# Leo-Liao-Chao/Uncertainty-Aware-CILQR-for-Trajectory-Optimization

Hardware: AMD Instinct MI355X
Metric: CILQR solves/sec (N=50, batch B) (higher is better)
Workload: dtype f64

## Files before the change

### uncertainty-aware-cilqr-for-trajectory-optimization_amd/csrc/cilqr_api.cpp

```cpp
#include <math.h>
#include <stdarg.h>
#include <stdio.h>
#include <stdlib.h>
#include <string.h>

#include <new>
#include <string>
#include <vector>

#include "cilqr_internal.h"

#include "cilqr_handle.h"

namespace cilqr {
thread_local std::string g_last_error;

int fail(int code, const char* fmt, ...) {
  char buf[512];
  va_list ap;
  va_start(ap, fmt);
  vsnprintf(buf, sizeof(buf), fmt, ap);
  va_end(ap);
  g_last_error = buf;
  return code;
// ... 2 lines not shown

using cilqr::fail;

namespace {

void derive(const cilqr_params& p, cilqr::KParams& k) {
  k.dt = p.timestep;
  k.desired_speed = p.desired_speed;
  k.tolerance = p.tolerance;
  k.w_acc = p.w_acc; k.w_yawrate = p.w_yawrate; k.w_pos = p.w_pos; k.w_vel = p.w_vel; k.w_obstacle = p.w_obstacle;
  k.q1_acc = p.q1_acc; k.q2_acc = p.q2_acc; k.q1_yawrate = p.q1_yawrate; k.q2_yawrate = p.q2_yawrate;
  k.q1_front = p.q1_front; k.q2_front = p.q2_front; k.q1_rear = p.q1_rear; k.q2_rear = p.q2_rear;
  k.acc_max = p.acc_max; k.acc_min = p.acc_min;
  k.yaw_hi = tan(p.steer_angle_max) / p.wheelbase;
  k.yaw_lo = tan(p.steer_angle_min) / p.wheelbase;
  k.half_dt2 = p.timestep * p.timestep / 2.0;
  k.wheelbase = p.wheelbase; k.speed_max = p.speed_max;
  k.t_safe = p.t_safe; k.s_safe_a = p.s_safe_a; k.s_safe_b = p.s_safe_b;
  k.ego_rad = p.ego_rad; k.ego_front = p.ego_front; k.ego_rear = p.ego_rear;
  k.lamb_factor = p.lamb_factor; k.lamb_max = p.lamb_max;
  k.max_iterations = p.max_iterations;
  k.n_samples = p.num_of_local_wpts * 10;
}

int check_sizes(const cilqr_handle* h, int B, int N, int M) {
  if (!h) return fail(CILQR_ERR_ARG, "null handle");
  if (B < 0 || B > h->max_batch) return fail(CILQR_ERR_ARG, "B=%d outside [0,%d]", B, h->max_batch);
  if (N < 1 || N > h->max_horizon) return fail(CILQR_ERR_ARG, "N=%d outside [1,%d]", N, h->max_horizon);
  if (M < 0 || M > h->max_obstacles) return fail(CILQR_ERR_ARG, "M=%d outside [0,%d]", M, h->max_obstacles);
  return CILQR_OK;
}

cilqr::SolveKnobs read_knobs(int simds) {
  const auto on = [](const char* name) { return getenv(name) != nullptr ? 1 : 0; };
  const auto num = [](const char* name, int unset) { const char* v = getenv(name); return v ? atoi(v) : unset; };
  cilqr::SolveKnobs k = {};
  k.simds = simds; k.force_g = num("CILQR_FORCE_G", 0);
  k.hint_off = on("CILQR_NO_SCHEDULE_HINT"); k.pair_on = on("CILQR_PAIR_KERNEL"); k.steal_off = on("CILQR_NO_LANE_SHARING"); k.split_off = on("CILQR_NO_SPLIT_KERNEL");
  k.share_off = on("CILQR_NO_SHARE_KERNEL"); k.tab_budget_kb = num("CILQR_LDS_TABLE_KB", 0);
  k.split_w = num("CILQR_SPLIT_W", 0);
  if (on("CILQR_SHARE_W")) k.share_w = num("CILQR_SHARE_W", 0) == 3 ? 3 : 2;
  k.share_max = num("CILQR_SHARE_MAX_B", -1);
  return k;
}

cilqr::SolveArgs handle_args(const cilqr_handle* h, int B, int N, int M, uint32_t flags) {
  cilqr::SolveArgs a = {};
  a.obs_tab = h->d_obs_tab; a.fwd = h->d_ws;
  a.redo = h->d_redo; a.diag = h->diag; a.passes = h->passes; a.unc = h->unc; a.kp = h->kp;
  a.B = B; a.N = N; a.M = M; a.flags = flags;
  return a;
}

template <typename T>
hipError_t dmalloc(T** p, size_t n) {
  *p = nullptr;
  if (n == 0) return hipSuccess;
  return hipMalloc((void**)p, n * sizeof(T));
}

int grow(float** p, size_t* cap, size_t n) {
  if (n <= *cap) return CILQR_OK;
  if (*p) HIP_TRY(hipFree(*p));
  *p = nullptr; *cap = 0;
  HIP_TRY(dmalloc(p, n));
  *cap = n;
  return CILQR_OK;
}

void set_obstacles(cilqr::SolveArgs& s, int M, const cilqr_obstacles* obs) {
  if (M <= 0) return;
  s.obs_pose = obs->pose; s.obs_dim = obs->dim; s.obs_weight = obs->weight;
  s.obs_bs = obs->batch_stride; s.obs_ms = obs->obstacle_stride; s.obs_ts = obs->step_stride; s.obs_wbs = obs->weight_batch_stride;
}

int check_sampled(const cilqr_handle* h, const char* name, int B, int N, int n_obs, int n_samples) {
  if (n_obs < 1 || n_samples < 2) return fail(CILQR_ERR_ARG, "%s: needs n_obs >= 1 and n_samples >= 2", name);
  if ((long)n_obs * n_samples > 1 << 20) return fail(CILQR_ERR_ARG, "%s: n_obs * n_samples too large", name);
  return check_sizes(h, B, N, n_obs * n_samples);
}

}

static int launch_wave_scheduled(cilqr_handle* h, cilqr::SolveArgs& a, const cilqr::WavePlan& plan, void* stream) {
  a.order = plan.hinted && h->hint_B == a.B && h->hint_stream == stream ? h->d_order : nullptr;
  a.hint_passes = plan.hinted ? h->d_hint_passes : nullptr;
  HIP_TRY(cilqr::launch_solve_wave(a, plan, (hipStream_t)stream));
  if (plan.hinted) {
    HIP_TRY(cilqr::launch_schedule_order(h->d_hint_passes, a.B, h->d_order, (hipStream_t)stream));
    h->hint_B = a.B; h->hint_stream = stream;
  }
  return CILQR_OK;
}

namespace {

int check_obstacles(int B, int N, int M, const cilqr_obstacles* o, size_t* span, size_t* w_span) {
  if (span) *span = 0;
  if (w_span) *w_span = 0;
  if (M == 0) return CILQR_OK;
  if (!o) return fail(CILQR_ERR_ARG, "cilqr_solve_batch_obstacles: M = %d but obs is null", M);
  if (!o->pose || !o->dim) return fail(CILQR_ERR_ARG, "cilqr_solve_batch_obstacles: M > 0 but obs->pose or obs->dim is null");
  if (o->batch_stride < 0 || o->obstacle_stride < 0 || o->step_stride < 0 || o->weight_batch_stride < 0)
    return fail(CILQR_ERR_ARG, "cilqr_solve_batch_obstacles: negative stride");
  const int64_t lim = (int64_t)1 << 40;
  if (o->batch_stride > lim || o->obstacle_stride > lim || o->step_stride > lim || o->weight_batch_stride > lim)
    return fail(CILQR_ERR_ARG, "cilqr_solve_batch_obstacles: stride beyond 2^40 entries");
  const int64_t b1 = B > 0 ? B - 1 : 0;
  if (span) *span = (size_t)(b1 * o->batch_stride + (int64_t)(M - 1) * o->obstacle_stride + (int64_t)(N - 1) * o->step_stride + 1);
  if (w_span && o->weight) *w_span = (size_t)(b1 * o->weight_batch_stride + M);
  return CILQR_OK;
}

int solve_device(cilqr_handle* h, void* stream, int B, int N, int M, const double* x0, double* U, const double* poly,
                 const double* xplan_fl, const cilqr_obstacles& o, double* X_out, double* J_out, int32_t* iters_out,
                 int32_t* status_out, uint32_t flags) {
  cilqr::SolveArgs a = handle_args(h, B, N, M, flags);
  a.x0 = x0; a.U = U; a.poly = poly; a.xplan_fl = xplan_fl;
  set_obstacles(a, M, &o);
  a.obs_shared = M > 0 && B > 1 && o.batch_stride == 0 && (!a.obs_weight || o.weight_batch_stride == 0) ? 1 : 0;
  a.X_out = X_out; a.J_out = J_out; a.iters_out = iters_out; a.status_out = status_out;
  a.steal = h->knobs.steal_off ? 0 : 1;
  HIP_TRY(hipSetDevice(h->device));
  const int G = cilqr::plan_group_lanes(h->knobs, B, N, M);
  if (G != 64) { HIP_TRY(cilqr::launch_solve_groups(a, G, h->d_ws, (hipStream_t)stream)); return CILQR_OK; }
  const cilqr::WavePlan plan = cilqr::plan_wave(h->knobs, {B, N, M, 0, h->kp.n_samples, flags, h->unc.layer != nullptr, a.obs_shared != 0});
  if (plan.too_large)
    return fail(CILQR_ERR_UNSUPPORTED, "cilqr_solve_batch: horizon %d needs %zu bytes of LDS per solve (limit %zu)", N, plan.lds_general, cilqr::SOLVE_LDS_MAX);
  return launch_wave_scheduled(h, a, plan, stream);
}

}

extern "C" {

int cilqr_abi_version(void) { return CILQR_ABI_VERSION; }

int cilqr_device_count(void) {
  int count = 0;
  if (hipGetDeviceCount(&count) != hipSuccess) return 0;
  int usable = 0;
  for (int d = 0; d < count; ++d) {
    hipDeviceProp_t prop;
    if (hipGetDeviceProperties(&prop, d) == hipSuccess && strncmp(prop.gcnArchName, "gfx950", 6) == 0) ++usable;
  }
  return usable;
}

const char* cilqr_last_error(void) { return cilqr::g_last_error.c_str(); }

void cilqr_params_default(cilqr_params* p) {
  if (!p) return;
  memset(p, 0, sizeof(*p));
  p->num_of_local_wpts = 20; p->poly_order = 5; p->desired_speed = 5.0;
  p->timestep = 0.1; p->horizon = 40; p->tolerance = 1e-4; p->max_iterations = 20;
  p->num_states = 4; p->num_ctrls = 2;
  p->w_acc = 1.0; p->w_yawrate = 4.0; p->w_pos = 0.65; p->w_vel = 3.0; p->w_obstacle = 1.0; p->w_uncertainty = 1.0;
  p->q1_acc = 1.0; p->q2_acc = 1.0; p->q1_yawrate = 1.0; p->q2_yawrate = 1.0;
  p->q1_front = 2.75; p->q2_front = 2.75; p->q1_rear = 2.5; p->q2_rear = 2.5;
  p->q1_uncertainty = 2.5; p->q2_uncertainty = 2.5;
  p->acc_max = 2.0; p->acc_min = -5.5; p->steer_angle_min = -0.75; p->steer_angle_max = 0.75;
  p->wheelbase = 2.94; p->speed_max = 30.0;
  p->steer_control_max = 1.0; p->steer_control_min = -1.0;
  p->throttle_control_max = 1.0; p->throttle_control_min = -1.0;
  p->t_safe = 0.1; p->s_safe_a = 0; p->s_safe_b = 0; p->ego_rad = 1.35;
  p->ego_front = 1.47 + 0.925; p->ego_rear = 1.47 + 0.925;
  p->length = 4.79; p->width = 2.16; p->safe_length = 0.0; p->safe_width = 0.0;
  p->lamb_factor = 10; p->lamb_max = 10000;
}

int cilqr_default_control_seq(int N, double* U) {
  if (N < 1 || !U) return fail(CILQR_ERR_ARG, "cilqr_default_control_seq: bad argument");
  const int num_zeros = N / 2;
  for (int i = 0; i < N; ++i) {
    U[2 * i] = 0.5;
    U[2 * i + 1] = i < num_zeros ? 0.0 : 0.1;
  }
  return CILQR_OK;
}

int cilqr_create(const cilqr_params* p, int max_batch, int max_horizon, int max_obstacles, int device,
                 cilqr_handle** out) {
  if (!p || !out) return fail(CILQR_ERR_ARG, "cilqr_create: null argument");
  *out = nullptr;
  if (max_batch < 1 || max_horizon < 1 || max_horizon > CILQR_MAX_HORIZON || max_obstacles < 0)
    return fail(CILQR_ERR_ARG, "cilqr_create: sizes out of range (max_horizon ≤ %d)", CILQR_MAX_HORIZON);
  if (p->num_states != CILQR_NX || p->num_ctrls != CILQR_NU || p->poly_order + 1 != CILQR_POLY_COEFFS)
    return fail(CILQR_ERR_UNSUPPORTED, "only num_states=4, num_ctrls=2, poly_order=5 are implemented (reference model, I/Model.cpp)");
  if (p->num_of_local_wpts < 1 || p->num_of_local_wpts > 100 || p->max_iterations < 1)
    return fail(CILQR_ERR_ARG, "cilqr_create: num_of_local_wpts / max_iterations out of range");
  int count = 0;
  hipError_t e = hipGetDeviceCount(&count);
  if (e != hipSuccess || count <= 0)
    return fail(CILQR_ERR_NO_DEVICE, "no HIP device available (%s); this library has no CPU path",
                e == hipSuccess ? "device count is 0" : hipGetErrorString(e));
  if (device < 0 || device >= count) return fail(CILQR_ERR_ARG, "device %d not in [0,%d)", device, count);
  hipDeviceProp_t prop;
  if (hipGetDeviceProperties(&prop, device) != hipSuccess) return fail(CILQR_ERR_NO_DEVICE, "hipGetDeviceProperties failed");
  if (strncmp(prop.gcnArchName, "gfx950", 6) != 0)
    return fail(CILQR_ERR_NO_DEVICE, "device %d is %s; this library is built for gfx950 only", device, prop.gcnArchName);
  if (hipSetDevice(device) != hipSuccess) return fail(CILQR_ERR_NO_DEVICE, "hipSetDevice(%d) failed", device);

  cilqr_handle* h = new (std::nothrow) cilqr_handle();
  if (!h) return fail(CILQR_ERR_ARG, "out of host memory");
  memset(h, 0, sizeof(*h));
  h->params = *p;
  derive(*p, h->kp);
  h->device = device;
  h->knobs = read_knobs(prop.multiProcessorCount > 0 ? prop.multiProcessorCount * 4 : 1024);
  h->max_batch = max_batch; h->max_horizon = max_horizon; h->max_obstacles = max_obstacles;
  const size_t B = max_batch, N = max_horizon, M = max_obstacles;
  hipError_t err = hipStreamCreateWithFlags(&h->stream, hipStreamNonBlocking);
  h->arena_cap = cilqr::host_arena_bytes(B, N, M);
  if (err == hipSuccess) err = hipMalloc((void**)&h->d_arena, h->arena_cap);
  h->stage_cap = h->arena_cap < ((size_t)1 << 20) ? h->arena_cap : ((size_t)1 << 20);
  if (err == hipSuccess) err = hipHostMalloc((void**)&h->stage, h->stage_cap, hipHostMallocDefault);
  const size_t Bpad = (B + 63) / 64 * 64;
  if (err == hipSuccess) err = dmalloc(&h->d_obs_tab, Bpad * M * N * 6);
  if (err == hipSuccess) err = dmalloc(&h->d_ws, cilqr::solve_groups_ws_doubles(max_batch, max_horizon));
  if (err == hipSuccess) err = dmalloc(&h->d_redo, B);
  if (err == hipSuccess) err = dmalloc(&h->d_hint_passes, B);
  if (err == hipSuccess) err = dmalloc(&h->d_order, B);
  h->hint_B = 0; h->hint_stream = nullptr;
  if (err == hipSuccess) err = dmalloc(&h->d_pair, (size_t)2);
  h->risk_part_stride = cilqr::RISK_PART_DOUBLES + (N + 1) / 2;
  if (err == hipSuccess) err = dmalloc(&h->d_risk_part, B * h->risk_part_stride);
  if (err == hipSuccess) err = dmalloc(&h->d_chance_map_steps, 3 * B * N);
  if (err == hipSuccess) err = dmalloc(&h->d_triple, (size_t)3);
  if (err == hipSuccess) err = dmalloc(&h->d_gather, (size_t)3);
  h->comm_ranks = 1;
  if (err == hipSuccess) err = dmalloc(&h->d_oob, (size_t)1);
  if (err == hipSuccess) err = dmalloc(&h->d_poses, (size_t)8 * 1024 * 4);
  if (err == hipSuccess) err = dmalloc(&h->d_polys, (size_t)8 * cilqr::POLYGON_TABLE_DOUBLES);
  if (err == hipSuccess) err = dmalloc(&h->d_occ_steps, (size_t)8 * 128);
  if (err == hipSuccess) {
    void* unused = nullptr;
    const size_t W = (size_t)p->num_of_local_wpts;
    if (cilqr::scratch_bytes(h, cilqr::SCR_PLAN_IO, (B * (4 + CILQR_POLY_COEFFS + 2 + 2 * W)) * sizeof(double) + B * sizeof(int32_t), &unused) != CILQR_OK ||
        cilqr::scratch_bytes(h, cilqr::SCR_PLAN_PATH, 2 * 1024 * sizeof(double), &unused) != CILQR_OK)
      err = hipErrorOutOfMemory;
  }
  if (err != hipSuccess) {
    int rc = fail(CILQR_ERR_HIP, "cilqr_create: device allocation failed: %s", hipGetErrorString(err));
    cilqr_destroy(h);
    return rc;
  }
  *out = h;
  return CILQR_OK;
}

int cilqr_destroy(cilqr_handle* h) {
  if (!h) return CILQR_OK;
  (void)hipSetDevice(h->device);
  if (h->stream) (void)hipStreamSynchronize(h->stream);
  (void)cilqr_comm_destroy(h);
  if (h->stage) (void)hipHostFree(h->stage);
  for (void* p : h->scratch)
    if (p) (void)hipFree(p);
  void* ptrs[] = {h->d_poses, h->d_polys, h->d_unc_layer, h->d_triple, h->d_gather, h->d_arena, h->d_obs_tab, h->d_ws, h->d_redo, h->d_hint_passes, h->d_order, h->d_pair, h->d_risk_part, h->d_chance_map_steps, h->d_src, h->d_dst, h->d_bbox, h->d_oob, h->d_occ_steps};
  for (void* p : ptrs)
    if (p) (void)hipFree(p);
  if (h->stream) (void)hipStreamDestroy(h->stream);
  delete h;
  return CILQR_OK;
}

int cilqr_set_diag_buffer(cilqr_handle* h, uint64_t* dev_buf) {
  if (!h) return fail(CILQR_ERR_ARG, "null handle");
  h->diag = (unsigned long long*)dev_buf;
  return CILQR_OK;
}

namespace {
int fill_unc(const cilqr_handle* h, const cilqr_uncertainty_map* m, cilqr::UncArgs& u) {
  if (!m || !m->layer) return fail(CILQR_ERR_ARG, "cilqr_set_uncertainty_map: null map or layer");
  const cilqr_map_geom& g = m->geom;
  if (g.rows < 2 || g.cols < 2 || !(g.res > 0.0) || !(g.len_x > 0.0) || !(g.len_y > 0.0))
    return fail(CILQR_ERR_ARG, "cilqr_set_uncertainty_map: bad geometry (needs at least 2x2 cells)");
  if (m->probes_l < 1 || m->probes_w < 1 || m->probes_l > 64 || m->probes_w > 64)
    return fail(CILQR_ERR_ARG, "cilqr_set_uncertainty_map: probes_l / probes_w must be in [1, 64]");
  if (m->layer_stride < 0 || (m->layer_stride > 0 && m->layer_stride < (int64_t)g.rows * g.cols))
    return fail(CILQR_ERR_ARG, "cilqr_set_uncertainty_map: layer_stride smaller than one layer");
  const cilqr_params& p = h->params;
  u.layer = m->layer;
  u.poses = m->poses;
  u.stride = m->layer_stride;
  u.rows = g.rows; u.cols = g.cols; u.nl = m->probes_l; u.nw = m->probes_w;
  u.x_first = g.pos_x + (0.5 * g.len_x - 0.5 * g.res);
  u.y_first = g.pos_y + (0.5 * g.len_y - 0.5 * g.res);
  u.inv_res = 1.0 / g.res;
  u.px = m->pose_x; u.py = m->pose_y;
  u.cp = cos(m->pose_theta);
  u.sp = sin(m->pose_theta);
  u.la0 = u.nl > 1 ? -0.5 * p.safe_length : 0.0;
  u.la_step = u.nl > 1 ? p.safe_length / (double)(u.nl - 1) : 0.0;
  u.wb0 = u.nw > 1 ? -0.5 * p.safe_width : 0.0;
  u.wb_step = u.nw > 1 ? p.safe_width / (double)(u.nw - 1) : 0.0;
  u.q1 = p.q1_uncertainty; u.q2 = p.q2_uncertainty;
  u.scale = p.w_uncertainty / (double)(u.nl * u.nw);
  return CILQR_OK;
}
}

int cilqr_set_uncertainty_map_device(cilqr_handle* h, const cilqr_uncertainty_map* map) {
  if (!h) return fail(CILQR_ERR_ARG, "null handle");
  cilqr::UncArgs u;
  int rc = fill_unc(h, map, u);
  if (rc) return rc;
  h->unc = u;
  return CILQR_OK;
}

int cilqr_set_uncertainty_map(cilqr_handle* h, const cilqr_uncertainty_map* map) {
  if (!h) return fail(CILQR_ERR_ARG, "null handle");
  if (map && (map->layer_stride != 0 || map->poses))
    return fail(CILQR_ERR_ARG, "cilqr_set_uncertainty_map: the host form takes one shared layer (per-solve layers / poses: use the _device form)");
  cilqr::UncArgs u;
  int rc = fill_unc(h, map, u);
  if (rc) return rc;
  HIP_TRY(hipSetDevice(h->device));
  const size_t n = (size_t)map->geom.rows * map->geom.cols;
  if (n > h->unc_layer_cap) {
    HIP_TRY(hipStreamSynchronize(h->stream));
    if (h->d_unc_layer) HIP_TRY(hipFree(h->d_unc_layer));
    h->d_unc_layer = nullptr; h->unc_layer_cap = 0;
    HIP_TRY(dmalloc(&h->d_unc_layer, n));
    h->unc_layer_cap = n;
  }
  HIP_TRY(hipMemcpyAsync(h->d_unc_layer, map->layer, n * sizeof(float), hipMemcpyHostToDevice, h->stream));
  HIP_TRY(hipStreamSynchronize(h->stream));
  u.layer = h->d_unc_layer;
  h->unc = u;
  return CILQR_OK;
}

int cilqr_clear_uncertainty_map(cilqr_handle* h) {
  if (!h) return fail(CILQR_ERR_ARG, "null handle");
  memset(&h->unc, 0, sizeof(h->unc));
  return CILQR_OK;
// ... 50 lines not shown
  HIP_TRY(hipMemcpyAsync(out, dout, sizeof(int32_t) * 3 * n, hipMemcpyDeviceToHost, h->stream));
  HIP_TRY(hipStreamSynchronize(h->stream));
  return CILQR_OK;
}

int cilqr_debug_blur_ellipse(cilqr_handle* h, int n, const double* abc, double* out) {
  if (!h || n < 1 || !abc || !out) return fail(CILQR_ERR_ARG, "cilqr_debug_blur_ellipse: bad argument");
  HIP_TRY(hipSetDevice(h->device));
  void* v = nullptr;
  int rc = cilqr::scratch_bytes(h, cilqr::SCR_DEBUG, sizeof(double) * 6 * (size_t)n, &v);
  if (rc) return rc;
  double *d_in = (double*)v, *d_out = d_in + 3 * (size_t)n;
  HIP_TRY(hipMemcpyAsync(d_in, abc, sizeof(double) * 3 * n, hipMemcpyHostToDevice, h->stream));
  HIP_TRY(cilqr::launch_blur_ellipse(n, d_in, d_out, h->stream));
  HIP_TRY(hipMemcpyAsync(out, d_out, sizeof(double) * 3 * n, hipMemcpyDeviceToHost, h->stream));
  HIP_TRY(hipStreamSynchronize(h->stream));
  return CILQR_OK;
}

int cilqr_wait(cilqr_handle* h) {
  if (!h) return fail(CILQR_ERR_ARG, "null handle");
  HIP_TRY(hipStreamSynchronize(h->stream));
  return CILQR_OK;
}

int cilqr_solve_family(const cilqr_handle* h, int B, int N, int M) {
  if (!h || B < 0 || N < 1 || M < 0) return fail(CILQR_ERR_ARG, "cilqr_solve_family: bad argument");
  return cilqr::plan_group_lanes(h->knobs, B, N, M);
}

int cilqr_solve_wavefronts(const cilqr_handle* h, int B, int N, int M) {
  if (!h || B < 0 || N < 1 || M < 0) return fail(CILQR_ERR_ARG, "cilqr_solve_wavefronts: bad argument");
  return cilqr::query_wavefronts(h->knobs, B, N, M, h->kp.n_samples, h->unc.layer != nullptr);
}

int cilqr_solve_sampled_wavefronts(const cilqr_handle* h, int B, int N, int n_obs) {
  if (!h || B < 0 || N < 1 || n_obs < 1) return fail(CILQR_ERR_ARG, "cilqr_solve_sampled_wavefronts: bad argument");
  return cilqr::split_shape_wavefronts(h->knobs, B, N, n_obs);
}

int cilqr_solve_batch_device(cilqr_handle* h, void* stream, int B, int N, int M, const double* x0, double* U,
                             const double* poly, const double* xplan_fl, const double* obs_pose, const double* obs_dim,
                             const double* obs_weight, double* X_out, double* J_out, int32_t* iters_out,
                             int32_t* status_out, uint32_t flags) {
  int rc = check_sizes(h, B, N, M);
  if (rc) return rc;
  if (B == 0) return CILQR_OK;
  if (!x0 || !U || !poly || !xplan_fl || !X_out) return fail(CILQR_ERR_ARG, "cilqr_solve_batch: null required pointer");
  if (M > 0 && (!obs_pose || !obs_dim)) return fail(CILQR_ERR_ARG, "cilqr_solve_batch: M > 0 but obstacle tables are null");
  const cilqr_obstacles o{obs_pose, obs_dim, obs_weight, (int64_t)M * N, N, 1, M};
  return solve_device(h, stream, B, N, M, x0, U, poly, xplan_fl, o, X_out, J_out, iters_out, status_out, flags);
}

int cilqr_solve_batch_obstacles_device(cilqr_handle* h, void* stream, int B, int N, int M, const double* x0, double* U,
                                       const double* poly, const double* xplan_fl, const cilqr_obstacles* obs, double* X_out,
                                       double* J_out, int32_t* iters_out, int32_t* status_out, uint32_t flags) {
  int rc = check_sizes(h, B, N, M);
  if (rc) return rc;
  rc = check_obstacles(B, N, M, obs, nullptr, nullptr);
  if (rc) return rc;
  if (B == 0) return CILQR_OK;
  if (!x0 || !U || !poly || !xplan_fl || !X_out) return fail(CILQR_ERR_ARG, "cilqr_solve_batch_obstacles: null required pointer");
  const cilqr_obstacles none{nullptr, nullptr, nullptr, 0, 0, 0, 0};
  return solve_device(h, stream, B, N, M, x0, U, poly, xplan_fl, M > 0 ? *obs : none, X_out, J_out, iters_out, status_out, flags);
}

}

int cilqr::host_solve_enqueue(cilqr_handle* h, int B, int N, int M, const double* x0, double* U, const double* poly, const double* xplan_fl,
                              const cilqr_obstacles* obs, size_t span, size_t w_span, double* X_out, double* J_out, int32_t* iters_out,
                              int32_t* status_out, uint32_t flags) {
  cilqr_obstacles o = M > 0 ? *obs : cilqr_obstacles{};
  const double* no_samples = nullptr;
  cilqr::HostPlan p(h->d_arena);
  cilqr::plan_solve(p, B, N, M, 0, x0, U, poly, xplan_fl, o, span, w_span, no_samples, X_out, J_out, iters_out, status_out);
  return cilqr::host_enqueue(h, p, [&] {
    const int rc = cilqr_solve_batch_obstacles_device(h, h->stream, B, N, M, x0, U, poly, xplan_fl, M > 0 ? &o : nullptr, X_out, J_out,
                                                      iters_out, status_out, flags);
    if (rc == CILQR_OK) h->d_J = J_out;
    return rc;
  }, true);
}

extern "C" {

int cilqr_solve_batch(cilqr_handle* h, int B, int N, int M, const double* x0, double* U, const double* poly,
                      const double* xplan_fl, const double* obs_pose, const double* obs_dim, const double* obs_weight,
                      double* X_out, double* J_out, int32_t* iters_out, int32_t* status_out, uint32_t flags) {
  int rc = check_sizes(h, B, N, M);
  if (rc) return rc;
  if (B == 0) return CILQR_OK;
  if (!x0 || !U || !poly || !xplan_fl || !X_out) return fail(CILQR_ERR_ARG, "cilqr_solve_batch: null required pointer");
  if (M > 0 && (!obs_pose || !obs_dim)) return fail(CILQR_ERR_ARG, "cilqr_solve_batch: M > 0 but obstacle tables are null");
  const cilqr_obstacles o{obs_pose, obs_dim, obs_weight, (int64_t)M * N, N, 1, M};
  rc = cilqr::host_solve_enqueue(h, B, N, M, x0, U, poly, xplan_fl, &o, (size_t)B * M * N, (size_t)B * M, X_out, J_out, iters_out, status_out, flags);
  return rc ? rc : cilqr::host_finish(h);
}

int cilqr_solve_batch_obstacles(cilqr_handle* h, int B, int N, int M, const double* x0, double* U, const double* poly,
                                const double* xplan_fl, const cilqr_obstacles* obs, double* X_out, double* J_out,
                                int32_t* iters_out, int32_t* status_out, uint32_t flags) {
  int rc = check_sizes(h, B, N, M);
  if (rc) return rc;
  size_t span = 0, w_span = 0;
  rc = check_obstacles(B, N, M, obs, &span, &w_span);
  if (rc) return rc;
  if (B == 0) return CILQR_OK;
  if (!x0 || !U || !poly || !xplan_fl || !X_out) return fail(CILQR_ERR_ARG, "cilqr_solve_batch_obstacles: null required pointer");
  rc = cilqr::host_solve_enqueue(h, B, N, M, x0, U, poly, xplan_fl, obs, span, w_span, X_out, J_out, iters_out, status_out, flags);
  return rc ? rc : cilqr::host_finish(h);
}

int cilqr_solve_batch_sampled_device(cilqr_handle* h, void* stream, int B, int N, int n_obs, int n_samples, const double* x0,
                                     double* U, const double* poly, const double* xplan_fl, const double* nom_pose,
                                     const double* nom_dim, const double* sample_offset, double sample_weight, double* X_out,
                                     double* J_out, int32_t* iters_out, int32_t* status_out, uint32_t flags) {
  int rc = check_sampled(h, "cilqr_solve_batch_sampled", B, N, n_obs, n_samples);
  if (rc) return rc;
  if (B == 0) return CILQR_OK;
  if (!x0 || !U || !poly || !xplan_fl || !X_out || !nom_pose || !nom_dim || !sample_offset)
    return fail(CILQR_ERR_ARG, "cilqr_solve_batch_sampled: null required pointer");
  const cilqr::WavePlan plan = cilqr::plan_wave(h->knobs, {B, N, n_obs, n_samples, h->kp.n_samples, flags, h->unc.layer != nullptr, false});
  if (plan.too_large)
    return fail(CILQR_ERR_UNSUPPORTED, "cilqr_solve_batch_sampled: n_obs * n_samples offset records do not fit LDS beside the solve");
  if (cilqr::sampled_tab_doubles(n_obs, N) > (size_t)h->max_obstacles * 6 * (size_t)h->max_horizon)
    return fail(CILQR_ERR_UNSUPPORTED, "cilqr_solve_batch_sampled: nominal records exceed the obstacle workspace reserved at create");
  cilqr::SolveArgs a = handle_args(h, B, N, n_obs, flags);
  a.x0 = x0; a.U = U; a.poly = poly; a.xplan_fl = xplan_fl;
  a.obs_pose = nom_pose; a.obs_dim = nom_dim;
  a.obs_bs = (long long)n_obs * N; a.obs_ms = N; a.obs_ts = 1;
  a.X_out = X_out; a.J_out = J_out; a.iters_out = iters_out; a.status_out = status_out;
  a.samp_off = sample_offset; a.n_samples = n_samples; a.samp_w = sample_weight;
  HIP_TRY(hipSetDevice(h->device));
  return launch_wave_scheduled(h, a, plan, stream);
}

int cilqr_solve_batch_sampled(cilqr_handle* h, int B, int N, int n_obs, int n_samples, const double* x0, double* U,
                              const double* poly, const double* xplan_fl, const double* nom_pose, const double* nom_dim,
                              const double* sample_offset, double sample_weight, double* X_out, double* J_out,
                              int32_t* iters_out, int32_t* status_out, uint32_t flags) {
  int rc = check_sampled(h, "cilqr_solve_batch_sampled", B, N, n_obs, n_samples);
  if (rc) return rc;
  if (B == 0) return CILQR_OK;
  if (!x0 || !U || !poly || !xplan_fl || !X_out || !nom_pose || !nom_dim || !sample_offset)
    return fail(CILQR_ERR_ARG, "cilqr_solve_batch_sampled: null required pointer");
  cilqr_obstacles o{nom_pose, nom_dim, nullptr, 0, 0, 0, 0};
  cilqr::HostPlan p(h->d_arena);
  cilqr::plan_solve(p, B, N, n_obs, n_samples, x0, U, poly, xplan_fl, o, (size_t)B * n_obs * N, 0, sample_offset, X_out, J_out, iters_out, status_out);
  return cilqr::host_call(h, p, [&] {
    const int rc = cilqr_solve_batch_sampled_device(h, h->stream, B, N, n_obs, n_samples, x0, U, poly, xplan_fl, o.pose, o.dim, sample_offset,
                                                    sample_weight, X_out, J_out, iters_out, status_out, flags);
    if (rc == CILQR_OK) h->d_J = J_out;
    return rc;
  }, true);
}

int cilqr_argmin_device(cilqr_handle* h, void* stream, int B, const double* J, double* out_pair) {
  if (!h || !J || !out_pair || B < 1) return fail(CILQR_ERR_ARG, "cilqr_argmin_device: bad argument");
  HIP_TRY(hipSetDevice(h->device));
  HIP_TRY(cilqr::launch_argmin(J, B, out_pair, nullptr, 0.0, (hipStream_t)stream));
  return CILQR_OK;
}

namespace {
int score_device(cilqr_handle* h, void* stream, cilqr::ScoreArgs& a, const double* X, const double* U, const double* poly,
                 const double* xplan_fl, double max_collision, double* score, double* total, int n_counters) {
  cilqr::SolveArgs& s = a.s;
  s.X_out = const_cast<double*>(X);
  s.U = const_cast<double*>(U);
  s.poly = poly; s.xplan_fl = xplan_fl;
  a.score = score; a.total = total; a.max_collision = max_collision; a.w_uncertainty = h->params.w_uncertainty;
  if (a.rows < 1) a.rows = 1;
  if (cilqr::score_lds_bytes(s.N, h->kp.n_samples, n_counters) > cilqr::SCORE_LDS_MAX)
    return fail(CILQR_ERR_UNSUPPORTED, "cilqr_score_batch: %d path samples, horizon %d and %d sample counters do not fit 64 KiB of LDS",
                h->kp.n_samples, s.N, n_counters);
  HIP_TRY(hipSetDevice(h->device));
  HIP_TRY(cilqr::launch_score(a, (hipStream_t)stream));
  return CILQR_OK;
}
}

int cilqr_score_batch_device(cilqr_handle* h, void* stream, int B, int N, int M, const double* X, const double* U, const double* poly,
                             const double* xplan_fl, const cilqr_obstacles* obs, double max_collision, double* score, double* total) {
  int rc = check_sizes(h, B, N, M);
  if (rc) return rc;
  rc = check_obstacles(B, N, M, obs, nullptr, nullptr);
  if (rc) return rc;
  if (!X || !U || !poly || !xplan_fl || !score) return fail(CILQR_ERR_ARG, "cilqr_score_batch: null required pointer");
  if ((int64_t)M * N > 0x7fffffff) return fail(CILQR_ERR_ARG, "cilqr_score_batch: M * N beyond 2^31 entries");
  if (B == 0) return CILQR_OK;
  cilqr::ScoreArgs a = {};
  a.s = handle_args(h, B, N, M, 0);
  set_obstacles(a.s, M, obs);
  return score_device(h, stream, a, X, U, poly, xplan_fl, max_collision, score, total, 0);
}

int cilqr_score_batch_sampled_device(cilqr_handle* h, void* stream, int B, int N, int n_obs, int n_samples, const double* X,
                                     const double* U, const double* poly, const double* xplan_fl, const double* nom_pose,
                                     const double* nom_dim, const double* sample_offset, double sample_weight, double max_collision,
                                     double* score, double* total) {
  int rc = check_sampled(h, "cilqr_score_batch_sampled", B, N, n_obs, n_samples);
  if (rc) return rc;
  if (!X || !U || !poly || !xplan_fl || !score || !nom_pose || !nom_dim || !sample_offset)
    return fail(CILQR_ERR_ARG, "cilqr_score_batch_sampled: null required pointer");
  if ((int64_t)n_obs * n_samples * N > 0x7fffffff) return fail(CILQR_ERR_ARG, "cilqr_score_batch_sampled: n_obs * n_samples * N beyond 2^31 entries");
  if (B == 0) return CILQR_OK;
  cilqr::ScoreArgs a = {};
  a.s = handle_args(h, B, N, n_obs, 0);
  a.s.obs_pose = nom_pose; a.s.obs_dim = nom_dim;
  a.s.samp_off = sample_offset; a.s.n_samples = n_samples; a.s.samp_w = sample_weight;
  return score_device(h, stream, a, X, U, poly, xplan_fl, max_collision, score, total, n_obs * N);
}

int cilqr_score_batch(cilqr_handle* h, int B, int N, int M, const double* X, const double* U, const double* poly,
                      const double* xplan_fl, const cilqr_obstacles* obs, double max_collision, double* score, double* total) {
  int rc = check_sizes(h, B, N, M);
  if (rc) return rc;
  size_t span = 0, w_span = 0;
  rc = check_obstacles(B, N, M, obs, &span, &w_span);
  if (rc) return rc;
  if (!X || !U || !poly || !xplan_fl || !score) return fail(CILQR_ERR_ARG, "cilqr_score_batch: null required pointer");
  if (B == 0) return CILQR_OK;
  cilqr_obstacles o = M > 0 ? *obs : cilqr_obstacles{};
  const double* no_samples = nullptr;
  cilqr::HostPlan p(h->d_arena);
  cilqr::plan_score(p, B, N, M, 0, X, U, poly, xplan_fl, o, span, w_span, no_samples, score, total);
  return cilqr::host_call(h, p, [&] {
    return cilqr_score_batch_device(h, h->stream, B, N, M, X, U, poly, xplan_fl, M > 0 ? &o : nullptr, max_collision, score, total);
  });
}

int cilqr_score_batch_sampled(cilqr_handle* h, int B, int N, int n_obs, int n_samples, const double* X, const double* U,
                              const double* poly, const double* xplan_fl, const double* nom_pose, const double* nom_dim,
                              const double* sample_offset, double sample_weight, double max_collision, double* score, double* total) {
  int rc = check_sampled(h, "cilqr_score_batch_sampled", B, N, n_obs, n_samples);
  if (rc) return rc;
  if (!X || !U || !poly || !xplan_fl || !score || !nom_pose || !nom_dim || !sample_offset)
// ... 1130 lines not shown
```

### uncertainty-aware-cilqr-for-trajectory-optimization_amd/csrc/cilqr_handle.h

```cpp
#pragma once

#include <string>

#include "cilqr_host_plan.h"
#include "cilqr_internal.h"

struct ncclComm;

struct cilqr_handle;

namespace cilqr {
struct PendingOut {
  bool active, packed;
  int n;
  HostPlan::Entry out[HostPlan::CAP];
};
int host_copy_in(cilqr_handle* h, const HostPlan& p, bool solve);
int host_copy_out(cilqr_handle* h, const HostPlan& p, int launch_rc);
int host_finish(cilqr_handle* h);
template <typename Launch>
int host_enqueue(cilqr_handle* h, const HostPlan& p, Launch&& launch, bool solve = false) {
  const int rc = host_copy_in(h, p, solve);
  return rc ? rc : host_copy_out(h, p, launch());
}
template <typename Launch>
int host_call(cilqr_handle* h, const HostPlan& p, Launch&& launch, bool solve = false) {
  const int rc = host_enqueue(h, p, launch, solve);
  return rc ? rc : host_finish(h);
}
int host_solve_enqueue(cilqr_handle* h, int B, int N, int M, const double* x0, double* U, const double* poly, const double* xplan_fl,
                       const cilqr_obstacles* obs, size_t span, size_t w_span, double* X_out, double* J_out, int32_t* iters_out,
                       int32_t* status_out, uint32_t flags);
enum { SCR_PLAN_PATH, SCR_PLAN_IO, SCR_COUNT, SCR_CONV_IN, SCR_CONV_OUT, SCR_DEBUG, SCR_SLOTS };
int scratch_bytes(cilqr_handle* h, int slot, size_t bytes, void** out);

extern thread_local std::string g_last_error;
int fail(int code, const char* fmt, ...);
}

#define HIP_TRY(expr)                                                                                      \
  do {                                                                                                     \
    hipError_t e_ = (expr);                                                                                \
    if (e_ != hipSuccess) return cilqr::fail(CILQR_ERR_HIP, "%s failed: %s", #expr, hipGetErrorString(e_)); \
  } while (0)

struct cilqr_handle {
  cilqr_params params;
  cilqr::KParams kp;
  int device;
  cilqr::SolveKnobs knobs;
  int max_batch, max_horizon, max_obstacles;
  hipStream_t stream;
  char* d_arena;
  size_t arena_cap;
  char* stage;
  size_t stage_cap;
  cilqr::PendingOut pending;
  int debug_fail_enqueue;
  double* d_J;
  void* scratch[cilqr::SCR_SLOTS];
  size_t scratch_cap[cilqr::SCR_SLOTS];
  double* d_obs_tab;
  double* d_ws;
  int32_t* d_redo;
  int32_t* d_hint_passes;
  int32_t* d_order;
  int hint_B;
  void* hint_stream;
  double* d_pair;
  double* d_risk_part;
  size_t risk_part_stride;
  double* d_chance_map_steps;
  float *d_src, *d_dst, *d_bbox;
  size_t src_cap, dst_cap, bbox_cap;
  unsigned long long* d_oob;
  double* d_poses;
  unsigned pose_slot;
  double* d_polys;
  unsigned poly_slot;
  float* d_occ_steps;
  unsigned occ_slot;
  unsigned long long* diag;
  int32_t* passes;
  cilqr::UncArgs unc;
  float* d_unc_layer;
  size_t unc_layer_cap;
  ncclComm* comm;
  int comm_ranks, comm_rank;
  double* d_triple;
  double* d_gather;
};
```

### uncertainty-aware-cilqr-for-trajectory-optimization_amd/csrc/cilqr_internal.h

```cpp
#pragma once

#include <hip/hip_runtime.h>
#include <stdint.h>

#include "cilqr.h"
#include "cilqr_wave_plan.h"

namespace cilqr {

struct KParams {
  double dt;
  double desired_speed;
  double tolerance;
  double w_acc, w_yawrate, w_pos, w_vel, w_obstacle;
  double q1_acc, q2_acc, q1_yawrate, q2_yawrate;
  double q1_front, q2_front, q1_rear, q2_rear;
  double acc_max, acc_min;
  double yaw_hi, yaw_lo;
  double half_dt2;
  double wheelbase, speed_max;
  double t_safe, s_safe_a, s_safe_b, ego_rad, ego_front, ego_rear;
  double lamb_factor, lamb_max;
  int32_t max_iterations;
  int32_t n_samples;
};

struct UncArgs {
  const float* layer;
  const double* poses;
  long long stride;
  int32_t rows, cols, nl, nw;
  double x_first, y_first, inv_res;
  double px, py, cp, sp;
  double la0, la_step, wb0, wb_step;
  double q1, q2, scale;
};

constexpr int DIAG_SLOTS = 16;

struct SolveArgs {
  const double* x0;
  double* U;
  const double* poly;
  const double* xplan_fl;
  const double* obs_pose;
  const double* obs_dim;
  const double* obs_weight;
  long long obs_bs, obs_ms, obs_ts, obs_wbs;
  int32_t obs_shared;
  double* X_out;
  double* J_out;
  int32_t* iters_out;
  int32_t* status_out;
  const double* samp_off;
  int32_t n_samples;
  double samp_w;
  double* obs_tab;
  double* fwd;
  int32_t* redo;
  unsigned long long* diag;
  int32_t* passes;
  const int32_t* order;
  int32_t* hint_passes;
  int32_t B, N, M;
  uint32_t flags;
  int32_t steal;
  KParams kp;
  UncArgs unc;
};

hipError_t launch_solve_wave(const SolveArgs& a, const WavePlan& plan, hipStream_t stream);
hipError_t launch_schedule_order(const int32_t* passes, int B, int32_t* order, hipStream_t stream);
hipError_t launch_solve_groups(const SolveArgs& a, int G, double* ws, hipStream_t stream);
size_t solve_groups_ws_doubles(int B, int N);
hipError_t launch_obstacle_table(const SolveArgs& a, hipStream_t stream);
hipError_t launch_unc_cost(const UncArgs& u, int n, const double* states, double* cost, double* vx, double* mx, hipStream_t stream);
hipError_t launch_quu_inverse(int n, const double* q, const double* lamb, double* out, int general, hipStream_t stream);
hipError_t launch_closest_sample(int n, int S, const double* in, int32_t* out, hipStream_t stream);

constexpr int SCORE_THREADS = 256;
constexpr size_t SCORE_LDS_MAX = 64 * 1024;
struct ScoreArgs {
  SolveArgs s;
  double* score;
  double* total;
  double max_collision;
  double w_uncertainty;
  int32_t rows;
};
hipError_t launch_score(const ScoreArgs& a, hipStream_t stream);
size_t score_lds_bytes(int N, int S, int n_counters);
struct RiskArgs {
  const double* row_score;
  double* risk;
  double* total;
  double max_risk;
  int32_t B, S;
};
hipError_t launch_risk(const RiskArgs& a, hipStream_t stream);

struct GainsArgs {
  SolveArgs s;
  double* k_out;
  double* K_out;
  int32_t* ok_out;
  double lamb;
};
hipError_t launch_gains(const GainsArgs& a, hipStream_t stream);
size_t gains_lds_bytes(int N, int n_path_samples);
constexpr size_t GAINS_LDS_MAX = 64 * 1024;

struct RolloutArgs {
  const double *X, *U, *k, *K;
  const double* delta;
  long long delta_bs;
  double* X_roll;
  double* U_roll;
  double k_scale;
  int32_t B, N, S;
  KParams kp;
};
hipError_t launch_rollout(const RolloutArgs& a, hipStream_t stream);
size_t rollout_lds_bytes(int N);

constexpr int RISK_THREADS = 256;
constexpr int RISK_WAVES = RISK_THREADS / 64;
constexpr int RISK_PART_DOUBLES = 8;
constexpr size_t RISK_LDS_MAX = 64 * 1024;
struct RolloutRiskArgs {
  SolveArgs s;
  const double *X, *U, *k, *K;
  const double* delta;
  long long delta_bs;
  double k_scale, max_risk;
  const double* base;
  double* risk;
  int32_t* step_hits;
  double* total;
  double* partials;
  long long part_stride;
  int32_t S, G;
};
hipError_t launch_rollout_risk(const RolloutRiskArgs& a, hipStream_t stream);
size_t rollout_risk_lds_bytes(int N, int M);
hipError_t launch_rollout_risk_sampled(const RolloutRiskArgs& a, hipStream_t stream);
size_t rollout_risk_sampled_lds_bytes(int N, int n_obs, int n_samples);
size_t rollout_risk_sampled_part_doubles(int N, int n_obs);
struct MapRiskArgs {
  RolloutRiskArgs r;
  double occ_threshold;
  int32_t* unknown_hits;
  uint32_t flags;
};
hipError_t launch_rollout_risk_map(const MapRiskArgs& a, hipStream_t stream);
// ... 129 lines not shown
```

### uncertainty-aware-cilqr-for-trajectory-optimization_amd/csrc/cilqr_solve.hip

```cpp
#include <type_traits>

#include "cilqr_device.hpp"

namespace cilqr {

using namespace dev;

namespace {

constexpr int FREC = 16;

__device__ __forceinline__ double readfirstlane_f64(double v) {
  int lo = __double2loint(v), hi = __double2hiint(v);
  lo = __builtin_amdgcn_readfirstlane(lo);
  hi = __builtin_amdgcn_readfirstlane(hi);
  return __hiloint2double(hi, lo);
}

__device__ __forceinline__ double wave_sum(double v) {
#pragma unroll
  for (int o = 32; o > 0; o >>= 1) v += __shfl_xor(v, o, WAVE);
  return v;
}

// ... 1676 lines not shown
  g.dmax = m;
  g.p2 = path_curvature_bound(g, pc, S, A, B);
  g.pc = pc;
  const double px = q[8], py = q[9];
  XWindow w = closest_window_x(S, g, px, py, at);
  closest_window_y(S, g, px, py, w);
  const int by_newton = w.hi - w.lo >= NEWTON_MIN_WINDOW ? closest_newton(S, g, px, py, at, w) : -1;
  out[3 * (size_t)i] = closest_sample(S, g, px, py, at);
  out[3 * (size_t)i + 1] = closest_scan(0, S - 1, px, py, at);
  out[3 * (size_t)i + 2] = by_newton >= 0 ? 1 : 0;
}

__global__ void unc_cost_kernel(UncArgs u, int n, const double* states, double* cost, double* vx, double* mx) {
  const int i = blockIdx.x * blockDim.x + threadIdx.x;
  if (i >= n) return;
  const UncPose po = unc_pose(u, 0);
  const double* st = states + 4 * (size_t)i;
  double sn, cs;
  sincos_fast(st[3], &sn, &cs);
  double g0 = 0.0, g1 = 0.0, h00 = 0.0, h01 = 0.0, h11 = 0.0;
  const double c = unc_cost_add(u, po, 0, st[0], st[1], cs, sn, g0, g1, h00, h01, h11);
  const double inv = u.scale != 0.0 ? 1.0 / (u.scale * (double)(u.nl * u.nw)) : 0.0;
  cost[i] = c;
  vx[2 * i] = g0 * inv; vx[2 * i + 1] = g1 * inv;
  mx[3 * i] = h00 * inv; mx[3 * i + 1] = h01 * inv; mx[3 * i + 2] = h11 * inv;
}

template <typename F>
hipError_t with_bool(bool b, F&& f) {
  return b ? f(std::true_type{}) : f(std::false_type{});
}
template <typename F>
hipError_t with_bools(bool b1, bool b2, F&& f) {
  return with_bool(b1, [&](auto c1) { return with_bool(b2, [&](auto c2) { return f(c1, c2); }); });
}

}

__global__ __launch_bounds__(1024) void schedule_order_kernel(const int32_t* passes, int B, int32_t* order) {
  __shared__ int cnt[64], base[64];
  const int tid = threadIdx.x;
  if (tid < 64) cnt[tid] = 0;
  __syncthreads();
  for (int i = tid; i < B; i += 1024) {
    const int p = passes[i];
    atomicAdd(&cnt[63 - (p < 0 ? 0 : p > 63 ? 63 : p)], 1);
  }
  __syncthreads();
  if (tid == 0) {
    int acc = 0;
    for (int k = 0; k < 64; ++k) { base[k] = acc; acc += cnt[k]; }
  }
  __syncthreads();
  for (int i = tid; i < B; i += 1024) {
    const int p = passes[i];
    order[atomicAdd(&base[63 - (p < 0 ? 0 : p > 63 ? 63 : p)], 1)] = i;
  }
}

hipError_t launch_schedule_order(const int32_t* passes, int B, int32_t* order, hipStream_t stream) {
  if (B <= 0) return hipSuccess;
  hipLaunchKernelGGL(schedule_order_kernel, dim3(1), dim3(1024), 0, stream, passes, B, order);
  return hipGetLastError();
}

hipError_t launch_unc_cost(const UncArgs& u, int n, const double* states, double* cost, double* vx, double* mx, hipStream_t stream) {
  if (n <= 0) return hipSuccess;
  hipLaunchKernelGGL(unc_cost_kernel, dim3((n + 63) / 64), dim3(64), 0, stream, u, n, states, cost, vx, mx);
  return hipGetLastError();
}

hipError_t launch_closest_sample(int n, int S, const double* in, int32_t* out, hipStream_t stream) {
  if (n <= 0) return hipSuccess;
  hipLaunchKernelGGL(closest_sample_kernel, dim3((n + 63) / 64), dim3(64), 0, stream, n, S, in, out);
  return hipGetLastError();
}

hipError_t launch_quu_inverse(int n, const double* q, const double* lamb, double* out, int general, hipStream_t stream) {
  if (n <= 0) return hipSuccess;
  hipLaunchKernelGGL(quu_inverse_kernel, dim3((n + 63) / 64), dim3(64), 0, stream, n, q, lamb, out, general);
  return hipGetLastError();
}

hipError_t launch_solve_wave(const SolveArgs& a, const WavePlan& p, hipStream_t stream) {
  if (a.B <= 0) return hipSuccess;
  if (p.too_large) return hipErrorInvalidValue;
  if (p.shared_table)
    if (const hipError_t e = launch_obstacle_table(a, stream)) return e;
  using Kernel = void (*)(SolveArgs);
  const auto go = [&](Kernel fast, Kernel general) {
    const size_t want = p.lds_fast > p.lds_general ? p.lds_fast : p.lds_general;
    hipError_t e = hipSuccess;
    for (Kernel k : {fast, general})
      if (want > SOLVE_LDS_DEFAULT && e == hipSuccess) e = hipFuncSetAttribute(reinterpret_cast<const void*>(k), hipFuncAttributeMaxDynamicSharedMemorySize, (int)want);
    void* args[] = {const_cast<SolveArgs*>(&a)};
    if (e == hipSuccess) e = hipLaunchKernel(reinterpret_cast<const void*>(fast), dim3(a.B), dim3(p.W * WAVE), args, p.lds_fast, stream);
    if (e == hipSuccess) e = hipLaunchKernel(reinterpret_cast<const void*>(general), dim3(a.B), dim3(WAVE), args, p.lds_general, stream);
    return e;
  };
  const bool diag = a.diag != nullptr, unc = a.unc.layer != nullptr;
  if (p.kernel == WavePlan::SPLIT)
    return with_bools(diag, unc, [&](auto d, auto u) {
      return p.W == 4 ? go(cilqr_solve_split_kernel<4, d.value, u.value>, cilqr_solve_kernel<d.value, 2, true, u.value>)
                      : go(cilqr_solve_split_kernel<2, d.value, u.value>, cilqr_solve_kernel<d.value, 2, true, u.value>);
    });
  if (p.tab == 2)
    return with_bools(diag, unc, [&](auto d, auto u) { return go(cilqr_solve_kernel<d.value, 2, false, u.value>, cilqr_solve_kernel<d.value, 2, true, u.value>); });
  if (p.kernel == WavePlan::PAIR)
    return with_bool(diag, [&](auto d) { return go(cilqr_solve_pair_kernel<d.value>, cilqr_solve_kernel<d.value, 1, true, false>); });
  if (p.kernel == WavePlan::SHARE)
    return with_bools(unc, diag, [&](auto u, auto d) {
      if (p.long_form) return go(cilqr_solve_share_kernel<2, true, d.value, u.value>, cilqr_solve_kernel<d.value, 1, true, u.value>);
      return p.W == 3 ? go(cilqr_solve_share_kernel<3, false, d.value, u.value>, cilqr_solve_kernel<d.value, 1, true, u.value>)
                      : go(cilqr_solve_share_kernel<2, false, d.value, u.value>, cilqr_solve_kernel<d.value, 1, true, u.value>);
    });
  return with_bool(diag, [&](auto d) {
    return p.tab == 1 ? with_bool(unc, [&](auto u) { return go(cilqr_solve_kernel<d.value, 1, false, u.value>, cilqr_solve_kernel<d.value, 1, true, u.value>); })
                      : with_bool(unc, [&](auto u) { return go(cilqr_solve_kernel<d.value, 0, false, u.value>, cilqr_solve_kernel<d.value, 0, true, u.value>); });
  });
}

}
```

Baseline: 2.487 million.

## Defer general-kernel launch on host path until fast pass hands off solves

On the host solve path, only the fast kernel runs first. After synchronizing, the host checks a mapped, coherent redo array and launches the general fallback kernel only when some batch entry was handed off. This is meant to skip the second kernel launch, which usually has nothing to do, at the cost of an extra host read and a possible second round-trip and sync. The grouped-lane path and the general-only or faithful-iters flags keep the single combined launch.

```diff
diff --git a/uncertainty-aware-cilqr-for-trajectory-optimization_amd/csrc/cilqr_api.cpp b/uncertainty-aware-cilqr-for-trajectory-optimization_amd/csrc/cilqr_api.cpp
--- a/uncertainty-aware-cilqr-for-trajectory-optimization_amd/csrc/cilqr_api.cpp
+++ b/uncertainty-aware-cilqr-for-trajectory-optimization_amd/csrc/cilqr_api.cpp
@@ -108,10 +108,15 @@
 
 }
 
-static int launch_wave_scheduled(cilqr_handle* h, cilqr::SolveArgs& a, const cilqr::WavePlan& plan, void* stream) {
+static int launch_wave_scheduled(cilqr_handle* h, cilqr::SolveArgs& a, const cilqr::WavePlan& plan, void* stream, int stage = cilqr::SOLVE_BOTH) {
+  if (stage != cilqr::SOLVE_BOTH) a.redo = h->redo_dev;
+  if (stage == cilqr::SOLVE_GENERAL) {
+    HIP_TRY(cilqr::launch_solve_wave(a, plan, (hipStream_t)stream, stage));
+    return CILQR_OK;
+  }
   a.order = plan.hinted && h->hint_B == a.B && h->hint_stream == stream ? h->d_order : nullptr;
   a.hint_passes = plan.hinted ? h->d_hint_passes : nullptr;
-  HIP_TRY(cilqr::launch_solve_wave(a, plan, (hipStream_t)stream));
+  HIP_TRY(cilqr::launch_solve_wave(a, plan, (hipStream_t)stream, stage));
   if (plan.hinted) {
     HIP_TRY(cilqr::launch_schedule_order(h->d_hint_passes, a.B, h->d_order, (hipStream_t)stream));
     h->hint_B = a.B; h->hint_stream = stream;
@@ -140,7 +145,7 @@
 
 int solve_device(cilqr_handle* h, void* stream, int B, int N, int M, const double* x0, double* U, const double* poly,
                  const double* xplan_fl, const cilqr_obstacles& o, double* X_out, double* J_out, int32_t* iters_out,
-                 int32_t* status_out, uint32_t flags) {
+                 int32_t* status_out, uint32_t flags, int stage = cilqr::SOLVE_BOTH) {
   cilqr::SolveArgs a = handle_args(h, B, N, M, flags);
   a.x0 = x0; a.U = U; a.poly = poly; a.xplan_fl = xplan_fl;
   set_obstacles(a, M, &o);
@@ -149,12 +154,49 @@
   a.steal = h->knobs.steal_off ? 0 : 1;
   HIP_TRY(hipSetDevice(h->device));
   const int G = cilqr::plan_group_lanes(h->knobs, B, N, M);
-  if (G != 64) { HIP_TRY(cilqr::launch_solve_groups(a, G, h->d_ws, (hipStream_t)stream)); return CILQR_OK; }
+  if (G != 64) {
+    if (stage != cilqr::SOLVE_BOTH) return fail(CILQR_ERR_ARG, "internal: the grouped family has no staged launch");
+    HIP_TRY(cilqr::launch_solve_groups(a, G, h->d_ws, (hipStream_t)stream));
+    return CILQR_OK;
+  }
   const cilqr::WavePlan plan = cilqr::plan_wave(h->knobs, {B, N, M, 0, h->kp.n_samples, flags, h->unc.layer != nullptr, a.obs_shared != 0});
   if (plan.too_large)
     return fail(CILQR_ERR_UNSUPPORTED, "cilqr_solve_batch: horizon %d needs %zu bytes of LDS per solve (limit %zu)", N, plan.lds_general, cilqr::SOLVE_LDS_MAX);
-  return launch_wave_scheduled(h, a, plan, stream);
-}
+  return launch_wave_scheduled(h, a, plan, stream, stage);
+}
+
+int solve_sampled_device(cilqr_handle* h, void* stream, int B, int N, int n_obs, int n_samples, const double* x0, double* U, const double* poly,
+                         const double* xplan_fl, const double* nom_pose, const double* nom_dim, const double* sample_offset,
+                         double sample_weight, double* X_out, double* J_out, int32_t* iters_out, int32_t* status_out, uint32_t flags,
+                         int stage = cilqr::SOLVE_BOTH) {
+  const cilqr::WavePlan plan = cilqr::plan_wave(h->knobs, {B, N, n_obs, n_samples, h->kp.n_samples, flags, h->unc.layer != nullptr, false});
+  if (plan.too_large)
+    return fail(CILQR_ERR_UNSUPPORTED, "cilqr_solve_batch_sampled: n_obs * n_samples offset records do not fit LDS beside the solve");
+  if (cilqr::sampled_tab_doubles(n_obs, N) > (size_t)h->max_obstacles * 6 * (size_t)h->max_horizon)
+    return fail(CILQR_ERR_UNSUPPORTED, "cilqr_solve_batch_sampled: nominal records exceed the obstacle workspace reserved at create");
+  cilqr::SolveArgs a = handle_args(h, B, N, n_obs, flags);
+  a.x0 = x0; a.U = U; a.poly = poly; a.xplan_fl = xplan_fl;
+  a.obs_pose = nom_pose; a.obs_dim = nom_dim;
+  a.obs_bs = (long long)n_obs * N; a.obs_ms = N; a.obs_ts = 1;
+  a.X_out = X_out; a.J_out = J_out; a.iters_out = iters_out; a.status_out = status_out;
+  a.samp_off = sample_offset; a.n_samples = n_samples; a.samp_w = sample_weight;
+  HIP_TRY(hipSetDevice(h->device));
+  return launch_wave_scheduled(h, a, plan, stream, stage);
+}
+
+template <typename Launch>
+int host_solve_run(cilqr_handle* h, const cilqr::HostPlan& p, int B, bool defer, Launch&& launch) {
+  int rc = cilqr::host_enqueue(h, p, [&] { return launch(defer ? cilqr::SOLVE_FIRST : cilqr::SOLVE_BOTH); }, true);
+  if (rc == CILQR_OK) rc = cilqr::host_finish(h);
+  if (rc || !defer) return rc;
+  int handed = 0;
+  for (int b = 0; b < B; ++b) handed += h->redo_host[b] != 0;
+  if (handed == 0) return CILQR_OK;
+  rc = cilqr::host_copy_out(h, p, launch(cilqr::SOLVE_GENERAL));
+  return rc ? rc : cilqr::host_finish(h);
+}
+
+bool host_defers_general(uint32_t flags) { return (flags & (CILQR_FLAG_GENERAL_ONLY | CILQR_FLAG_FAITHFUL_ITERS)) == 0; }
 
 }
 
@@ -249,6 +291,8 @@
   if (err == hipSuccess) err = dmalloc(&h->d_order, B);
   h->hint_B = 0; h->hint_stream = nullptr;
   if (err == hipSuccess) err = dmalloc(&h->d_pair, (size_t)2);
+  if (err == hipSuccess) err = hipHostMalloc((void**)&h->redo_host, B * sizeof(int32_t), hipHostMallocMapped | hipHostMallocCoherent);
+  if (err == hipSuccess) err = hipHostGetDevicePointer((void**)&h->redo_dev, h->redo_host, 0);
   h->risk_part_stride = cilqr::RISK_PART_DOUBLES + (N + 1) / 2;
   if (err == hipSuccess) err = dmalloc(&h->d_risk_part, B * h->risk_part_stride);
   if (err == hipSuccess) err = dmalloc(&h->d_chance_map_steps, 3 * B * N);
@@ -281,6 +325,7 @@
   if (h->stream) (void)hipStreamSynchronize(h->stream);
   (void)cilqr_comm_destroy(h);
   if (h->stage) (void)hipHostFree(h->stage);
+  if (h->redo_host) (void)hipHostFree(h->redo_host);
   for (void* p : h->scratch)
     if (p) (void)hipFree(p);
   void* ptrs[] = {h->d_poses, h->d_polys, h->d_unc_layer, h->d_triple, h->d_gather, h->d_arena, h->d_obs_tab, h->d_ws, h->d_redo, h->d_hint_passes, h->d_order, h->d_pair, h->d_risk_part, h->d_chance_map_steps, h->d_src, h->d_dst, h->d_bbox, h->d_oob, h->d_occ_steps};
@@ -497,6 +542,23 @@
   }, true);
 }
 
+namespace {
+int host_solve(cilqr_handle* h, int B, int N, int M, const double* x0, double* U, const double* poly, const double* xplan_fl,
+               const cilqr_obstacles* obs, size_t span, size_t w_span, double* X_out, double* J_out, int32_t* iters_out, int32_t* status_out,
+               uint32_t flags) {
+  cilqr_obstacles o = M > 0 ? *obs : cilqr_obstacles{};
+  const double* no_samples = nullptr;
+  cilqr::HostPlan p(h->d_arena);
+  cilqr::plan_solve(p, B, N, M, 0, x0, U, poly, xplan_fl, o, span, w_span, no_samples, X_out, J_out, iters_out, status_out);
+  const bool defer = host_defers_general(flags) && cilqr::plan_group_lanes(h->knobs, B, N, M) == 64;
+  return host_solve_run(h, p, B, defer, [&](int stage) {
+    const int rc = solve_device(h, h->stream, B, N, M, x0, U, poly, xplan_fl, o, X_out, J_out, iters_out, status_out, flags, stage);
+    if (rc == CILQR_OK) h->d_J = J_out;
+    return rc;
+  });
+}
+}
+
 extern "C" {
 
 int cilqr_solve_batch(cilqr_handle* h, int B, int N, int M, const double* x0, double* U, const double* poly,
@@ -508,8 +570,7 @@
   if (!x0 || !U || !poly || !xplan_fl || !X_out) return fail(CILQR_ERR_ARG, "cilqr_solve_batch: null required pointer");
   if (M > 0 && (!obs_pose || !obs_dim)) return fail(CILQR_ERR_ARG, "cilqr_solve_batch: M > 0 but obstacle tables are null");
   const cilqr_obstacles o{obs_pose, obs_dim, obs_weight, (int64_t)M * N, N, 1, M};
-  rc = cilqr::host_solve_enqueue(h, B, N, M, x0, U, poly, xplan_fl, &o, (size_t)B * M * N, (size_t)B * M, X_out, J_out, iters_out, status_out, flags);
-  return rc ? rc : cilqr::host_finish(h);
+  return host_solve(h, B, N, M, x0, U, poly, xplan_fl, &o, (size_t)B * M * N, (size_t)B * M, X_out, J_out, iters_out, status_out, flags);
 }
 
 int cilqr_solve_batch_obstacles(cilqr_handle* h, int B, int N, int M, const double* x0, double* U, const double* poly,
@@ -522,8 +583,7 @@
   if (rc) return rc;
   if (B == 0) return CILQR_OK;
   if (!x0 || !U || !poly || !xplan_fl || !X_out) return fail(CILQR_ERR_ARG, "cilqr_solve_batch_obstacles: null required pointer");
-  rc = cilqr::host_solve_enqueue(h, B, N, M, x0, U, poly, xplan_fl, obs, span, w_span, X_out, J_out, iters_out, status_out, flags);
-  return rc ? rc : cilqr::host_finish(h);
+  return host_solve(h, B, N, M, x0, U, poly, xplan_fl, obs, span, w_span, X_out, J_out, iters_out, status_out, flags);
 }
 
 int cilqr_solve_batch_sampled_device(cilqr_handle* h, void* stream, int B, int N, int n_obs, int n_samples, const double* x0,
@@ -535,19 +595,8 @@
   if (B == 0) return CILQR_OK;
   if (!x0 || !U || !poly || !xplan_fl || !X_out || !nom_pose || !nom_dim || !sample_offset)
     return fail(CILQR_ERR_ARG, "cilqr_solve_batch_sampled: null required pointer");
-  const cilqr::WavePlan plan = cilqr::plan_wave(h->knobs, {B, N, n_obs, n_samples, h->kp.n_samples, flags, h->unc.layer != nullptr, false});
-  if (plan.too_large)
-    return fail(CILQR_ERR_UNSUPPORTED, "cilqr_solve_batch_sampled: n_obs * n_samples offset records do not fit LDS beside the solve");
-  if (cilqr::sampled_tab_doubles(n_obs, N) > (size_t)h->max_obstacles * 6 * (size_t)h->max_horizon)
-    return fail(CILQR_ERR_UNSUPPORTED, "cilqr_solve_batch_sampled: nominal records exceed the obstacle workspace reserved at create");
-  cilqr::SolveArgs a = handle_args(h, B, N, n_obs, flags);
-  a.x0 = x0; a.U = U; a.poly = poly; a.xplan_fl = xplan_fl;
-  a.obs_pose = nom_pose; a.obs_dim = nom_dim;
-  a.obs_bs = (long long)n_obs * N; a.obs_ms = N; a.obs_ts = 1;
-  a.X_out = X_out; a.J_out = J_out; a.iters_out = iters_out; a.status_out = status_out;
-  a.samp_off = sample_offset; a.n_samples = n_samples; a.samp_w = sample_weight;
-  HIP_TRY(hipSetDevice(h->device));
-  return launch_wave_scheduled(h, a, plan, stream);
+  return solve_sampled_device(h, stream, B, N, n_obs, n_samples, x0, U, poly, xplan_fl, nom_pose, nom_dim, sample_offset, sample_weight, X_out,
+                              J_out, iters_out, status_out, flags);
 }
 
 int cilqr_solve_batch_sampled(cilqr_handle* h, int B, int N, int n_obs, int n_samples, const double* x0, double* U,
@@ -562,12 +611,12 @@
   cilqr_obstacles o{nom_pose, nom_dim, nullptr, 0, 0, 0, 0};
   cilqr::HostPlan p(h->d_arena);
   cilqr::plan_solve(p, B, N, n_obs, n_samples, x0, U, poly, xplan_fl, o, (size_t)B * n_obs * N, 0, sample_offset, X_out, J_out, iters_out, status_out);
-  return cilqr::host_call(h, p, [&] {
-    const int rc = cilqr_solve_batch_sampled_device(h, h->stream, B, N, n_obs, n_samples, x0, U, poly, xplan_fl, o.pose, o.dim, sample_offset,
-                                                    sample_weight, X_out, J_out, iters_out, status_out, flags);
+  return host_solve_run(h, p, B, host_defers_general(flags), [&](int stage) {
+    const int rc = solve_sampled_device(h, h->stream, B, N, n_obs, n_samples, x0, U, poly, xplan_fl, o.pose, o.dim, sample_offset, sample_weight,
+                                        X_out, J_out, iters_out, status_out, flags, stage);
     if (rc == CILQR_OK) h->d_J = J_out;
     return rc;
-  }, true);
+  });
 }
 
 int cilqr_argmin_device(cilqr_handle* h, void* stream, int B, const double* J, double* out_pair) {
diff --git a/uncertainty-aware-cilqr-for-trajectory-optimization_amd/csrc/cilqr_handle.h b/uncertainty-aware-cilqr-for-trajectory-optimization_amd/csrc/cilqr_handle.h
--- a/uncertainty-aware-cilqr-for-trajectory-optimization_amd/csrc/cilqr_handle.h
+++ b/uncertainty-aware-cilqr-for-trajectory-optimization_amd/csrc/cilqr_handle.h
@@ -68,6 +68,7 @@
   int hint_B;
   void* hint_stream;
   double* d_pair;
+  int32_t *redo_host, *redo_dev;
   double* d_risk_part;
   size_t risk_part_stride;
   double* d_chance_map_steps;
diff --git a/uncertainty-aware-cilqr-for-trajectory-optimization_amd/csrc/cilqr_internal.h b/uncertainty-aware-cilqr-for-trajectory-optimization_amd/csrc/cilqr_internal.h
--- a/uncertainty-aware-cilqr-for-trajectory-optimization_amd/csrc/cilqr_internal.h
+++ b/uncertainty-aware-cilqr-for-trajectory-optimization_amd/csrc/cilqr_internal.h
@@ -69,7 +69,8 @@
   UncArgs unc;
 };
 
-hipError_t launch_solve_wave(const SolveArgs& a, const WavePlan& plan, hipStream_t stream);
+enum { SOLVE_BOTH, SOLVE_FIRST, SOLVE_GENERAL };
+hipError_t launch_solve_wave(const SolveArgs& a, const WavePlan& plan, hipStream_t stream, int stage = SOLVE_BOTH);
 hipError_t launch_schedule_order(const int32_t* passes, int B, int32_t* order, hipStream_t stream);
 hipError_t launch_solve_groups(const SolveArgs& a, int G, double* ws, hipStream_t stream);
 size_t solve_groups_ws_doubles(int B, int N);
diff --git a/uncertainty-aware-cilqr-for-trajectory-optimization_amd/csrc/cilqr_solve.hip b/uncertainty-aware-cilqr-for-trajectory-optimization_amd/csrc/cilqr_solve.hip
--- a/uncertainty-aware-cilqr-for-trajectory-optimization_amd/csrc/cilqr_solve.hip
+++ b/uncertainty-aware-cilqr-for-trajectory-optimization_amd/csrc/cilqr_solve.hip
@@ -1782,10 +1782,10 @@
   return hipGetLastError();
 }
 
-hipError_t launch_solve_wave(const SolveArgs& a, const WavePlan& p, hipStream_t stream) {
+hipError_t launch_solve_wave(const SolveArgs& a, const WavePlan& p, hipStream_t stream, int stage) {
   if (a.B <= 0) return hipSuccess;
   if (p.too_large) return hipErrorInvalidValue;
-  if (p.shared_table)
+  if (p.shared_table && stage != SOLVE_GENERAL)
     if (const hipError_t e = launch_obstacle_table(a, stream)) return e;
   using Kernel = void (*)(SolveArgs);
   const auto go = [&](Kernel fast, Kernel general) {
@@ -1794,8 +1794,8 @@
     for (Kernel k : {fast, general})
       if (want > SOLVE_LDS_DEFAULT && e == hipSuccess) e = hipFuncSetAttribute(reinterpret_cast<const void*>(k), hipFuncAttributeMaxDynamicSharedMemorySize, (int)want);
     void* args[] = {const_cast<SolveArgs*>(&a)};
-    if (e == hipSuccess) e = hipLaunchKernel(reinterpret_cast<const void*>(fast), dim3(a.B), dim3(p.W * WAVE), args, p.lds_fast, stream);
-    if (e == hipSuccess) e = hipLaunchKernel(reinterpret_cast<const void*>(general), dim3(a.B), dim3(WAVE), args, p.lds_general, stream);
+    if (e == hipSuccess && stage != SOLVE_GENERAL) e = hipLaunchKernel(reinterpret_cast<const void*>(fast), dim3(a.B), dim3(p.W * WAVE), args, p.lds_fast, stream);
+    if (e == hipSuccess && stage != SOLVE_FIRST) e = hipLaunchKernel(reinterpret_cast<const void*>(general), dim3(a.B), dim3(WAVE), args, p.lds_general, stream);
     return e;
   };
   const bool diag = a.diag != nullptr, unc = a.unc.layer != nullptr;
```

After: 2.487 million, median of 2. About the same (-0.0%).
